# Tilka/hvqm4

Hardware: AMD Instinct MI355X
Metric: decoded Mpixels/s (bit-exact YUV) (higher is better)
Workload: dtype u8

## Files before the change

### hvqm4_amd/csrc/hvq_kernels.hip

```cpp
#include <hip/hip_runtime.h>
#include <stdint.h>
#include <algorithm>

#include "hvq_desc.h"
#include "../../include/hvqm4_amd.h"

typedef uint32_t u32;
typedef int32_t i32;
typedef uint64_t __attribute__((aligned(1))) u64u;
#define GLB __attribute__((address_space(1)))
typedef short s16x2 __attribute__((ext_vector_type(2)));
typedef unsigned short u16x2 __attribute__((ext_vector_type(2)));

#define HVQ_WG HVQ_TILE_BLOCKS
#ifndef HVQ_MIN_WAVES
#define HVQ_MIN_WAVES 8
#endif

struct Blk { u32 r[4]; };

__device__ __forceinline__ u32 sat_pack(s16x2 a, s16x2 b)
{
    const u16x2 k255 = { 255, 255 };
    u16x2 ua = __builtin_elementwise_min(__builtin_bit_cast(u16x2, (s16x2)(a >> 3)), k255);
// ... 27 lines not shown
#pragma unroll
    for (int y = 0; y < 4; ++y) r.q[y] = *(const GLB u64u *)(ref + a + y * stride);
    r.q[4] = 0;
    if (hy) r.q[4] = *(const GLB u64u *)(ref + a + 4 * stride);
    return r;
}

__device__ __forceinline__ Blk mc_filter(const McRows &rows, int hx, int hy)
{
    const uint64_t *q = rows.q;
    Blk o;
    u32 hp, xp;
    {
        const u32 p = (u32)q[0], n = hx ? (u32)(q[0] >> 8) : p;
        hp = __builtin_amdgcn_lerp(p, n, 0u); xp = p ^ n;
    }
#pragma unroll
    for (int y = 0; y < 4; ++y) {
        const u32 p = (u32)q[y + 1], n = hx ? (u32)(q[y + 1] >> 8) : p;
        const u32 hn = __builtin_amdgcn_lerp(p, n, 0u), xn = p ^ n;
        const u32 h1 = hy ? hn : hp, x1 = hy ? xn : xp;
        const u32 t = __builtin_amdgcn_lerp(hp, h1, 0x01010101u);
        o.r[y] = t + (xp & x1 & ~(hp ^ h1) & 0x01010101u);
        hp = hn; xp = xn;
    }
    return o;
}


template <int N>
__device__ __forceinline__ u32 udiv_table(u32 den)
{
    const u32 q = (u32)__builtin_fmaf(__builtin_amdgcn_rcpf((float)den), (float)N, 0.0009765625f);
    return den ? q : 0u;
}

__device__ __forceinline__ i32 sar(u32 v, i32 s)
{
    i32 r = (i32)v >> s;
    __asm__ volatile("" : "+v"(r));
    return r;
}

__device__ __forceinline__ u32 basis_gain(u32 d, u32 lo, u32 hi)
{
    const u32 q = udiv_table<256>((hi - lo) & 15u);
    const u32 s = d >> 14;
    const u32 g = s * (q << 4);
    return (d & 0x2000u) ? 0u - g : g;
}

template <int STRIDE>
__device__ __forceinline__ void basis_scatter(u32 g, const u32 e[16], u32 *acc_lds)
{
#if defined(HVQ_ABL) && HVQ_ABL == 5
    u32 t = 0;
#pragma unroll
    for (int i = 0; i < 16; ++i) t ^= g * e[i];
    __hip_atomic_fetch_add(acc_lds, t, __ATOMIC_RELAXED, __HIP_MEMORY_SCOPE_WORKGROUP);
#else
#pragma unroll
    for (int i = 0; i < 16; ++i)
        __hip_atomic_fetch_add(acc_lds + i * STRIDE, g * e[i], __ATOMIC_RELAXED, __HIP_MEMORY_SCOPE_WORKGROUP);
#endif
}

__device__ __forceinline__ u32 shr_sat_pack4(u32 a, u32 b, u32 c, u32 d, i32 s)
{
    const u32 lo = (u32)__builtin_amdgcn_ashr_pk_u8_i32((i32)a, (i32)b, (u32)s);
    const u32 hi = (u32)__builtin_amdgcn_ashr_pk_u8_i32((i32)c, (i32)d, (u32)s);
    return __builtin_amdgcn_perm(hi, lo, 0x05040100u);
}

__device__ __forceinline__ Blk intra_finish(const u32 r[16], i32 V, i32 unk)
{
    u32 total = 0;
#pragma unroll
    for (int i = 0; i < 16; ++i) total += r[i];
    const u32 delta = ((u32)V << unk) - (u32)((i32)total >> 4);
    Blk o4;
#pragma unroll
    for (int y = 0; y < 4; ++y)
        o4.r[y] = shr_sat_pack4(r[4 * y] + delta, r[4 * y + 1] + delta, r[4 * y + 2] + delta, r[4 * y + 3] + delta, unk);
    return o4;
}

__device__ __forceinline__ Blk predi_finish(const u32 r[16], Blk m, u32 p0, u32 p1, i32 unk)
{
    u32 total = 0;
#pragma unroll
    for (int i = 0; i < 16; ++i) total += r[i];
    const u32 mean_aot = (u32)((i32)total >> 4);
    u32 sum = 8;
#pragma unroll
    for (int y = 0; y < 4; ++y) sum = __builtin_amdgcn_sad_u8(m.r[y], 0u, sum);
    const u32 mean = sum >> 4;
    u32 lo = 255, hi = 0;
#pragma unroll
    for (int y = 0; y < 4; ++y)
#pragma unroll
        for (int x = 0; x < 4; ++x) {
            const u32 v = (m.r[y] >> (8 * x)) & 0xFFu;
            lo = min(lo, v);
            hi = max(hi, v);
        }
    const u32 mcd = udiv_table<4096>(hi - lo);
    const u32 factor = p1 * mcd;
    const u32 c = p0 - mean_aot - mean * factor;
    Blk o4;
#pragma unroll
    for (int y = 0; y < 4; ++y) {
        u32 v[4];
#pragma unroll
        for (int x = 0; x < 4; ++x) {
            const u32 px = (m.r[y] >> (8 * x)) & 0xFFu;
            v[x] = (u32)(((i32)(r[4 * y + x] + c + px * factor) >> unk) + (i32)px);
        }
        o4.r[y] = shr_sat_pack4(v[0], v[1], v[2], v[3], 0);
    }
    return o4;
}

__device__ __forceinline__ u32 wave_incl_scan(u32 v)
{
    v += (u32)__builtin_amdgcn_update_dpp(0, (int)v, 0x111, 0xF, 0xF, false);
    v += (u32)__builtin_amdgcn_update_dpp(0, (int)v, 0x112, 0xF, 0xF, false);
    v += (u32)__builtin_amdgcn_update_dpp(0, (int)v, 0x114, 0xF, 0xF, false);
    v += (u32)__builtin_amdgcn_update_dpp(0, (int)v, 0x118, 0xF, 0xF, false);
    v += (u32)__builtin_amdgcn_update_dpp(0, (int)v, 0x142, 0xA, 0xF, false);
    v += (u32)__builtin_amdgcn_update_dpp(0, (int)v, 0x143, 0xC, 0xF, false);
    return v;
}

__device__ __forceinline__ u32 lanes_below(unsigned long long mask)
{
    return __builtin_amdgcn_mbcnt_hi((u32)(mask >> 32), __builtin_amdgcn_mbcnt_lo((u32)mask, 0u));
}

#define HVQ_NW (HVQ_WG / 64)
#ifndef HVQ_ABL
#define HVQ_ABL 0
#endif
#ifndef HVQ_NT_LOADS
#define HVQ_NT_LOADS 0
#endif
#ifndef HVQ_PRIO
#define HVQ_PRIO 0
#endif
#ifndef HVQ_PLANE_LOAD
#define HVQ_PLANE_LOAD 1
#endif
#ifndef HVQ_NT_STORES
#define HVQ_NT_STORES 1
#endif

#ifdef HVQ_STAMPS
static unsigned long long *g_stamps = nullptr;
extern "C" __attribute__((visibility("default"))) void hvq_set_stamps(unsigned long long *p) { g_stamps = p; }
#define HVQ_STAMP_ARG , unsigned long long *stamps
#define STAMP(i, VM) do { unsigned long long t_; __builtin_amdgcn_sched_barrier(0); \
        if (VM) asm volatile("s_waitcnt vmcnt(0)" ::: "memory"); \
        asm volatile("s_memtime %0\n\ts_waitcnt lgkmcnt(0)" : "=s"(t_) :: "memory"); __builtin_amdgcn_sched_barrier(0); \
        if (stamps && (threadIdx.x & 63) == 0) stamps[(((size_t)blockIdx.z * gridDim.y + blockIdx.y) * gridDim.x + blockIdx.x) * 64 + (threadIdx.x >> 6) * 16 + (i)] = t_; } while (0)
#else
#define HVQ_STAMP_ARG
#define STAMP(i, VM) do { } while (0)
#endif

typedef u32 u32x2 __attribute__((ext_vector_type(2)));
#define HVQ_PIN(x) do { x = (u32)__builtin_amdgcn_readfirstlane((int)(x)); asm("" : "+s"(x)); } while (0)

struct SrGeo {
    GLB uint8_t *pic;
    i32 lim;
};
__device__ __forceinline__ u32 sr_ld(const SrGeo &g, i32 o)
{
    o = clampi(o, 0, g.lim);
    return __hip_atomic_load(g.pic + o, __ATOMIC_RELAXED, __HIP_MEMORY_SCOPE_AGENT);
}
__device__ __forceinline__ void sr_st(const SrGeo &g, i32 o, u32 v)
{
    o = clampi(o, 0, g.lim);
    __hip_atomic_store(g.pic + o, (uint8_t)v, __ATOMIC_RELAXED, __HIP_MEMORY_SCOPE_AGENT);
}
__device__ __forceinline__ u32 sr_mc_sample(const SrGeo &g, i32 so, i32 stride, int hx, int hy, int i, int j)
{
    const i32 a = so + i * stride + j;
    if (!hx && !hy) return sr_ld(g, a);
    if (hx && !hy) return (sr_ld(g, a) + sr_ld(g, a + 1) + 1u) / 2u;
    if (!hx) return (sr_ld(g, a) + sr_ld(g, a + stride) + 1u) / 2u;
    return (sr_ld(g, a) + sr_ld(g, a + 1) + sr_ld(g, a + stride) + sr_ld(g, a + stride + 1) + 2u) >> 2;
}

__global__ __launch_bounds__(HVQ_WG)
void hvq_selfref_kernel(const HvqJob *__restrict__ J, const uint8_t *__restrict__ side, uint8_t *pic)
{
    const int tid = threadIdx.x;
    const u32 flags = J->flags;
    const bool is15 = flags & HVQ_F_IS15, landscape = flags & HVQ_F_LANDSCAPE;
    const i32 unk = (i32)((flags >> HVQ_JOB_UNK_SHIFT) & 31u);
    const i32 lw = (i32)J->width, mcb_w = (i32)J->mcb_w;
    const i32 nmb = mcb_w * (i32)((J->plane[0].hbvb >> 16) / 2u);
    const GLB u32 *__restrict__ pool = (const GLB u32 *)J->pool;
    const GLB u32 *__restrict__ mvs = (const GLB u32 *)J->mv;
    const GLB u32 *__restrict__ offs = (const GLB u32 *)((const GLB uint8_t *)J->tq + J->q_offs_off);
    SrGeo g;
    g.pic = (GLB uint8_t *)pic;
    g.lim = (i32)J->slot_bytes - 1;
    struct { const GLB uint8_t *map; i32 hb, pw, ws, hs, poff; u32 tile_first; } P[3];
#pragma unroll
    for (int k = 0; k < 3; ++k) {
        P[k].map = (const GLB uint8_t *)J->plane[k].map;
        P[k].hb = (i32)(J->plane[k].hbvb & 0xFFFFu);
        P[k].pw = (i32)(J->plane[k].pw_sub & 0xFFFFu);
        P[k].ws = (i32)((J->plane[k].pw_sub >> 16) & 0xFFu); P[k].hs = (i32)(J->plane[k].pw_sub >> 24);
        P[k].poff = (i32)J->plane[k].plane_off;
        P[k].tile_first = J->plane[k].tile_first;
    }
    bool moved = false;
    for (i32 m = 0; m < nmb; ++m) {
        const i32 my = m / mcb_w, mx = m - my * mcb_w;
        const u32 T = (u32)__builtin_amdgcn_readfirstlane((int)P[0].map[2 * ((2 * my + 1) * (P[0].hb + 2) + 2 * mx + 1) + 1]);
        if (((T >> 5) & 3u) != 2u) {
            int k = -1, r = 0, col = 0;
            const int cw = 8 >> P[1].ws, ch = 8 >> P[1].hs, cn = cw * ch;
            if (tid < 64) { k = 0; r = tid >> 3; col = tid & 7; }
            else if (tid - 64 < cn) { k = 1; r = (tid - 64) / cw; col = (tid - 64) - r * cw; }
            else if (tid - 64 - cn < cn) { k = 2; r = (tid - 64 - cn) / cw; col = (tid - 64 - cn) - r * cw; }
            if (k >= 0) {
                const i32 o = P[k].poff + (my * (8 >> P[k].hs) + r) * P[k].pw + mx * (8 >> P[k].ws) + col;
                pic[o] = side[o];
            }
            moved = true;
            continue;
        }
        if (moved) { __syncthreads(); moved = false; }
        if (tid == 0) {
            const u32 mvw = mvs[m];
            const i32 rx = (i32)(int16_t)(mvw & 0xFFFF), ry = (i32)(int16_t)(mvw >> 16);
            const bool proc = T & 0x10u;
            const i32 origin = landscape ? rx / 2 + (ry / 2 - 16) * lw - 32 : rx / 2 + (ry / 2 - 32) * lw - 16;
            for (int k = 0; k < 3; ++k) {
                const i32 pw = P[k].pw, ws = P[k].ws, hs = P[k].hs;
                const i32 pdx = rx >> ws, pdy = ry >> hs;
                const int hx = is15 ? (pdx & 1) : (rx & 1), hy = is15 ? (pdy & 1) : (ry & 1);
                const int bxp = 2 >> ws, byp = 2 >> hs, nblk = bxp * byp;
                for (int j = 0; j < nblk; ++j) {
                    const int dx = nblk == 1 ? 0 : (j >> 1), dy = nblk == 1 ? 0 : ((j == 1 || j == 2) ? 1 : 0);
                    const i32 bx = mx * bxp + dx, by = my * byp + dy;
                    const i32 dsto = P[k].poff + by * 4 * pw + bx * 4;
                    const i32 srco = P[k].poff + (pdy >> 1) * pw + (pdx >> 1) + dy * 4 * pw + dx * 4;
                    const u32 kind = (u32)P[k].map[2 * ((by + 1) * (P[k].hb + 2) + bx + 1) + 1] & 0xFu;
                    const u32 b = (u32)(by * P[k].hb + bx);
                    const u32 off = offs[(size_t)(P[k].tile_first + b / HVQ_TILE_BLOCKS) * HVQ_TILE_BLOCKS + b % HVQ_TILE_BLOCKS];
                    if (!proc && kind == 6u) {
                        for (int i = 0; i < 4; ++i) {
                            const u32 w4 = pool[off + (u32)i];
                            for (int x = 0; x < 4; ++x) sr_st(g, dsto + i * pw + x, (w4 >> (8 * x)) & 0xFFu);
                        }
                    } else if (proc || kind == 0u) {
                        for (int i = 0; i < 4; ++i)
                            for (int x = 0; x < 4; ++x) sr_st(g, dsto + i * pw + x, sr_mc_sample(g, srco, pw, hx, hy, i, x));
                    } else {
                        u32 acc[16];
                        for (int i = 0; i < 16; ++i) acc[i] = 0;
                        const u32 nb = kind - 1u;
                        for (u32 q = 0; q < nb; ++q) {
                            const u32 d = pool[off + 2u + q];
                            const i32 ol = d & 0x3F, os = (d >> 6) & 0x1F;
                            const u32 sl = (d >> 11) & 1, ss = (d >> 12) & 1;
                            i32 o, ys, xs;
                            if (landscape) { o = lw * os + ol; xs = 1 << sl; ys = lw << ss; }
                            else           { o = lw * ol + os; xs = 1 << ss; ys = lw << sl; }
                            u32 e[16], lo = 255, hi = 0;
                            for (int i = 0; i < 4; ++i)
                                for (int x = 0; x < 4; ++x) {
                                    const u32 v = (sr_ld(g, origin + o + i * ys + x * xs) >> 4) & 15u;
                                    e[4 * i + x] = v; lo = min(lo, v); hi = max(hi, v);
                                }
                            const u32 gn = basis_gain(d, lo, hi);
                            for (int i = 0; i < 16; ++i) acc[i] += gn * e[i];
                        }
                        u32 total = 0;
                        for (int i = 0; i < 16; ++i) total += acc[i];
                        const u32 mean_aot = (u32)((i32)total >> 4);
                        u32 md[16], sum = 8, lo = 255, hi = 0;
                        for (int i = 0; i < 4; ++i)
                            for (int x = 0; x < 4; ++x) { const u32 v = sr_mc_sample(g, srco, pw, hx, hy, i, x); md[4 * i + x] = v; sum += v; lo = min(lo, v); hi = max(hi, v); }
                        const i32 mean = (i32)(sum >> 4);
                        const u32 addend = pool[off] - mean_aot;
                        const u32 factor = pool[off + 1u] * udiv_table<4096>(hi - lo);
                        for (int i = 0; i < 16; ++i) {
                            const u32 t = (u32)((i32)md[i] - mean) * factor;
                            const i32 v = sar(acc[i] + addend + t, unk) + (i32)md[i];
                            sr_st(g, dsto + (i >> 2) * pw + (i & 3), (u32)clampi(v, 0, 255));
                        }
                    }
                }
            }
        }
        __syncthreads();
    }
}

extern "C" hipError_t hvq_launch_selfref(const HvqJob *job_dev, const uint8_t *side, uint8_t *dst, hipStream_t stream)
{
    hipLaunchKernelGGL(hvq_selfref_kernel, dim3(1), dim3(HVQ_WG), 0, stream, job_dev, side, dst);
    return hipGetLastError();
}

__device__ __forceinline__ u32 gain_q(u32 w0, u32 lo, u32 hi)
{
    const u32 q = udiv_table<256>((hi - lo) & 15u);
    const u32 g = (w0 & 0x3FFFFu) * (q << 4);
    return (w0 & HVQ_PQ_NEG) ? 0u - g : g;
}

__device__ __forceinline__ void gather_nest_q(i32 o, bool x2, i32 ys, const uint8_t *s_nest, u32 e[16], u32 &lo, u32 &hi)
{
    const u32 sh = x2 ? 8u : 4u;
    lo = 255; hi = 0;
#pragma unroll
    for (int y = 0; y < 4; ++y) {
        const i32 n = o + y * ys;
        uint64_t q = *(const u64u *)(s_nest + (n >> 1));
        q >>= 4 * (n & 1);
        const u32 w0 = (u32)q;
#pragma unroll
        for (int x = 0; x < 4; ++x) {
            u32 v = (w0 >> (sh * x)) & 15u;
            e[4 * y + x] = v;
            lo = min(lo, v);
            hi = max(hi, v);
        }
    }
}

__device__ __forceinline__ void window_load(const GLB uint8_t *ring, u32 voff, u32 ys, uint64_t q[4])
{
    if (HVQ_ABL == 19) { q[0] = *(const GLB u64u *)(ring + (size_t)voff); q[1] = *(const GLB u64u *)(ring + (size_t)(u32)(voff + ys)); q[2] = q[0] ^ 1; q[3] = q[1] ^ 1; return; }
    if (HVQ_ABL == 20) { q[0] = *(const GLB u64u *)(ring + (size_t)voff); q[1] = q[0] ^ 1; q[2] = q[0] ^ 2; q[3] = q[1] ^ 3; return; }
    if (HVQ_ABL == 21) voff &= 0xFFFFu;
#pragma unroll
    for (int y = 0; y < 4; ++y) q[y] = *(const GLB u64u *)(ring + (size_t)(u32)(voff + (u32)y * ys));
}

__device__ __forceinline__ void window_finish(const uint64_t q[4], bool x2, u32 e[16], u32 &lo, u32 &hi)
{
    const u32 sel = x2 ? 0x06040200u : 0x03020100u;
    lo = 255; hi = 0;
#pragma unroll
    for (int y = 0; y < 4; ++y) {
        u32 w = __builtin_amdgcn_perm((u32)(q[y] >> 32), (u32)q[y], sel);
        w = (w >> 4) & 0x0F0F0F0Fu;
#pragma unroll
        for (int x = 0; x < 4; ++x) {
            u32 v = (w >> (8 * x)) & 0xFFu;
            e[4 * y + x] = v;
            lo = min(lo, v);
            hi = max(hi, v);
        }
    }
}


template <int CTX>
__device__ __forceinline__ void inl_classify(u32 T, bool valid, u32 &cls, u32 &nb, u32 &npay, bool &lit, bool &mc, bool &wdc, bool &flat)
{
    const u32 kind = CTX == 0 ? T : (T & 0xFu);
    const bool k0 = kind == 0u, k6 = kind == 6u, k8 = kind == 8u;
    if (CTX == 2) {
        const bool inter = T & 0x60u, proc = T & 0x10u;
        const bool c1 = valid && !inter && !(k0 | k6 | k8), c2 = valid && inter && !proc && !(k0 | k6);
        lit = valid && k6 && !(inter && proc);
        mc = valid && inter && (proc || !k6); wdc = valid && !inter && k0; flat = valid && !inter && k8;
        cls = c1 ? 1u : c2 ? 2u : 0u;
        nb = c1 ? kind : c2 ? kind - 1u : 0u;
        npay = lit ? 4u : nb + (c2 ? 2u : 0u);
    } else {
        const bool c1 = valid && !(k0 | k6 | k8);
        lit = valid && k6; mc = false; wdc = valid && k0; flat = valid && k8;
        cls = c1 ? 1u : 0u; nb = c1 ? kind : 0u; npay = lit ? 4u : nb;
    }
}

template <int N> struct InlCtx { static constexpr int value = N; };
#define HVQ_W64(i) ((uint64_t)cw[i] | ((uint64_t)cw[(i) + 1] << 32))

constexpr u32 HVQ_INL_NEST_LDS = (HVQ_NESTP_BYTES + 8 + 15) / 16 * 16;
constexpr u32 HVQ_INL_ACC_DW = 16, HVQ_INL_RES_DW = 4, HVQ_INL_REC_DW = 3;
constexpr u32 HVQ_INL_CTR_LDS = 16;
constexpr u32 hvq_inl_static_lds(u32 items_cap)
{
    return HVQ_INL_NEST_LDS + 4u * (HVQ_INL_ACC_DW + HVQ_INL_RES_DW + HVQ_INL_REC_DW) * items_cap + HVQ_INL_CTR_LDS;
}
#ifndef HVQ_SEVEN_WG_CAP
#define HVQ_SEVEN_WG_CAP 128
#endif
constexpr int hvq_inl_waves(int tpw, int items_cap) { return (tpw >= 2 && items_cap >= HVQ_SEVEN_WG_CAP) ? 7 : HVQ_MIN_WAVES; }
template <int ITEMS_CAP, int TPW> struct InlWaves { static constexpr int value = hvq_inl_waves(TPW, ITEMS_CAP); };

template <int ITEMS_CAP, int TPW>
__global__ __launch_bounds__(HVQ_WG, (InlWaves<ITEMS_CAP, TPW>::value))
void hvq_recon_inline_kernel(const HvqJob *__restrict__ jobs, u32 pair_cap, u32 pool_cap HVQ_STAMP_ARG)
{
    extern __shared__ __attribute__((aligned(16))) u32 s_dyn[];
    __shared__ __attribute__((aligned(16))) uint8_t s_nest[HVQ_INL_NEST_LDS];
    __shared__ __attribute__((aligned(16))) u32 s_acc[HVQ_INL_ACC_DW * ITEMS_CAP];
    __shared__ __attribute__((aligned(16))) u32 s_res[HVQ_INL_RES_DW * ITEMS_CAP];
    __shared__ u32 s_item0[ITEMS_CAP];
    __shared__ u32 s_item1[ITEMS_CAP];
    __shared__ u32 s_item2[ITEMS_CAP];
    __shared__ __attribute__((aligned(16))) unsigned long long s_ctr64;
    static_assert(sizeof(s_nest) + sizeof(s_acc) + sizeof(s_res) + sizeof(s_item0) + sizeof(s_item1) + sizeof(s_item2) + HVQ_INL_CTR_LDS == hvq_inl_static_lds(ITEMS_CAP)
                  && ITEMS_CAP % 4 == 0 && sizeof(s_ctr64) <= HVQ_INL_CTR_LDS, "the host sizes launches by hvq_inl_static_lds");
    u32 *const s_pair = s_dyn;
    u32 *const s_pool = s_dyn + pair_cap;

    const int tid = threadIdx.x;
    const u32 lane = (u32)tid & 63u;
    STAMP(0, 0);
#if HVQ_PRIO == 1 || HVQ_PRIO == 2
    __builtin_amdgcn_s_setprio(3);
#endif
    const u32 slot_id = blockIdx.z * gridDim.x + blockIdx.x;
    const u32 wg = blockIdx.y;
    const HvqJob *__restrict__ J = jobs + slot_id;
#if HVQ_PLANE_LOAD
    const u32 *__restrict__ CW = (const u32 *)J;
    u32 cw[20];
#pragma unroll
    for (int i = 0; i < 20; ++i) cw[i] = CW[i];
    u32 wb_lo = CW[46], wb_hi = CW[47], q_offs_off = CW[49];
#pragma unroll
    for (int i = 0; i < 20; ++i) HVQ_PIN(cw[i]);
    HVQ_PIN(wb_lo); HVQ_PIN(wb_hi); HVQ_PIN(q_offs_off);
    const u32 total_tiles = cw[17];
    const u32 n0 = cw[18], n1 = cw[19] - cw[18], n2 = total_tiles - cw[19];
    const u32 pf1 = (n0 + TPW - 1) / TPW, pf2 = pf1 + (n1 + TPW - 1) / TPW, pend = pf2 + (n2 + TPW - 1) / TPW;
    if (total_tiles == 0 || wg >= pend) return;
    const int p = (wg >= pf1) + (wg >= pf2);
    const u32 *__restrict__ PW = CW + 20 + 8 * p;
    u32 w[8];
#pragma unroll
    for (int i = 0; i < 8; ++i) w[i] = PW[i];
    u32 magic = CW[52 + p], magic16 = CW[55 + p];
#pragma unroll
    for (int i = 0; i < 8; ++i) HVQ_PIN(w[i]);
    HVQ_PIN(magic); HVQ_PIN(magic16);
#else
    const u32 *__restrict__ PW = (const u32 *)&J->plane[0];
    u32 w0[8], w1[8], w2[8];
#pragma unroll
    for (int i = 0; i < 8; ++i) { w0[i] = PW[i]; w1[i] = PW[8 + i]; w2[i] = PW[16 + i]; }
    const u32 *__restrict__ CW = (const u32 *)J;
    u32 cw[18];
#pragma unroll
    for (int i = 0; i < 18; ++i) cw[i] = CW[i];
    u32 wb_lo = CW[46], wb_hi = CW[47], q_offs_off = CW[49];
    u32 mg0 = CW[52], mg1 = CW[53], mg2 = CW[54], ms0 = CW[55], ms1 = CW[56], ms2 = CW[57];
#pragma unroll
    for (int i = 0; i < 8; ++i) { HVQ_PIN(w0[i]); HVQ_PIN(w1[i]); HVQ_PIN(w2[i]); }
#pragma unroll
    for (int i = 0; i < 18; ++i) HVQ_PIN(cw[i]);
    HVQ_PIN(wb_lo); HVQ_PIN(wb_hi); HVQ_PIN(q_offs_off);
    HVQ_PIN(mg0); HVQ_PIN(mg1); HVQ_PIN(mg2); HVQ_PIN(ms0); HVQ_PIN(ms1); HVQ_PIN(ms2);
    const u32 total_tiles = cw[17];
    const u32 n0 = w1[5] - w0[5], n1 = w2[5] - w1[5], n2 = total_tiles - w2[5];
    const u32 pf1 = (n0 + TPW - 1) / TPW, pf2 = pf1 + (n1 + TPW - 1) / TPW, pend = pf2 + (n2 + TPW - 1) / TPW;
    if (total_tiles == 0 || wg >= pend) return;
    const int p = (wg >= pf1) + (wg >= pf2);
    u32 w[8];
#pragma unroll
    for (int i = 0; i < 8; ++i) w[i] = p == 0 ? w0[i] : p == 1 ? w1[i] : w2[i];
    const u32 magic = p == 0 ? mg0 : p == 1 ? mg1 : mg2, magic16 = p == 0 ? ms0 : p == 1 ? ms1 : ms2;
#endif
    const u32 hbvb = w[6], pw_sub = w[7], tile_first = w[5];
    const u32 nplane_tiles = p == 0 ? n0 : p == 1 ? n1 : n2;
    const u32 pairw = wg - (p == 0 ? 0u : p == 1 ? pf1 : pf2);
    const u32 tile0 = tile_first + (u32)TPW * pairw;
    const int ntl = TPW == 1 ? 1 : (int)min((u32)TPW, nplane_tiles - (u32)TPW * pairw);
    const uint64_t map_a = (uint64_t)w[0] | ((uint64_t)w[1] << 32);
    const uint64_t dst_a = (uint64_t)w[2] | ((uint64_t)w[3] << 32);
    const u32 plane_off = w[4];
    const u32 hb = hbvb & 0xFFFFu;
    const u32 flags = cw[13];
    const u32 pic_kind = (flags >> HVQ_JOB_KIND_SHIFT) & 3u;
    const i32 unk = (i32)((flags >> HVQ_JOB_UNK_SHIFT) & 31u);
    const bool is_pb = pic_kind != HVQ_PIC_I;
    const bool landscape = flags & HVQ_F_LANDSCAPE;
    const bool is15 = flags & HVQ_F_IS15;
    const u32 nblocks = hb * (hbvb >> 16);
    const u32 b0 = (u32)TPW * pairw * HVQ_TILE_BLOCKS;
    const u32 ws = (pw_sub >> 16) & 0xFFu, hs = pw_sub >> 24;
    const u32 pw = pw_sub & 0xFFFFu;
    const u32 mstride = hb + 2u;
    const GLB uint8_t *map = (const GLB uint8_t *)map_a;
    const GLB uint8_t *ring = (const GLB uint8_t *)HVQ_W64(0);
    const u32 ref0_off = cw[2], ref1_off = cw[3];
    const GLB u32 *__restrict__ pool = (const GLB u32 *)HVQ_W64(4);
    const GLB u32 *__restrict__ mvs = (const GLB u32 *)HVQ_W64(6);
    const GLB uint8_t *__restrict__ qb = (const GLB uint8_t *)HVQ_W64(8);
    const GLB u32 *__restrict__ nestp = (const GLB u32 *)HVQ_W64(10);
    const GLB u32 *__restrict__ wave_base = (const GLB u32 *)((uint64_t)wb_lo | ((uint64_t)wb_hi << 32));
    GLB uint8_t *plane = (GLB uint8_t *)dst_a;
    const i32 slot = (i32)cw[12];
    const u32 lw = cw[14];
    const u32 mcb_w = cw[15];
    const u32 pool_dwords = cw[16];
    const u32 wave = (u32)__builtin_amdgcn_readfirstlane(tid >> 6);
    STAMP(1, 0);
    if (tid == 0) s_ctr64 = 0;
    __syncthreads();

    u32 plo = wave_base[tile0 * HVQ_NW];
    u32 phi = tile0 + (u32)ntl < total_tiles ? wave_base[(tile0 + (u32)ntl) * HVQ_NW] : pool_dwords;
    u32 wbase[TPW];
#pragma unroll
    for (int h = 0; h < TPW; ++h) wbase[h] = h < ntl ? wave_base[(tile0 + (u32)h) * HVQ_NW + wave] : 0u;
    bool valid[TPW];
    u32 bx[TPW], by[TPW];
    uint64_t row8[TPW];
    u32 nt[TPW], nbt[TPW], mvw[TPW];
    Blk blk[TPW];
    u32 doff[TPW], rslot[TPW];
#pragma unroll
    for (int h = 0; h < TPW; ++h) {
        const u32 bw = b0 + (u32)(h * HVQ_TILE_BLOCKS) + wave * 64u;
        const bool livew = h < ntl && bw < nblocks;
        valid[h] = h < ntl && bw + lane < nblocks;
        const u32 bws = livew ? bw : 0u;
        u32 by0 = __umulhi(bws, magic);
        if ((i32)(bws - by0 * hb) < 0) by0 -= 1u;
        const u32 bx0 = bws - by0 * hb;
        const u32 l = valid[h] ? lane : 0u;
        const u32 t = bx0 + l;
        u32 q;
        if (hb >= 64u) q = t >= hb ? 1u : 0u;
        else q = __umul24(t, magic16) >> 16;
        bx[h] = t - __umul24(q, hb); by[h] = by0 + q;
        doff[h] = valid[h] ? __umul24(by[h] << 2, pw) + (bx[h] << 2) : 0xFFFFFFFFu;
        const GLB uint8_t *mw = map + 2u * (size_t)(bws + 2u * by0 + hb + 3u);
        const u32 vo2 = 2u * (l + 2u * q);
#if HVQ_NT_LOADS
        row8[h] = __builtin_nontemporal_load((const GLB u64u *)((mw - 2) + vo2));
#else
        row8[h] = *(const GLB u64u *)((mw - 2) + vo2);
#endif
        if (HVQ_ABL >= 41 && HVQ_ABL <= 43) { nt[h] = (u32)row8[h] & 0xFFFFu; nbt[h] = (u32)(row8[h] >> 32) & 0xFFFFu; }
        else { nt[h] = *(const GLB uint16_t *)((mw - 2u * (size_t)mstride) + vo2); nbt[h] = *(const GLB uint16_t *)((mw + 2u * (size_t)mstride) + vo2); }
        mvw[h] = 0;
        if (HVQ_ABL == 42 || HVQ_ABL == 43) { if (is_pb) { const u32 hh = ((bx[h] >> (1u - ws)) * 73u + (by[h] >> (1u - hs)) * 151u) * 2654435761u; mvw[h] = (((hh >> 8) & 1023u) + 16u) | ((((hh >> 18) & 511u) + 64u) << 16); } }
        else if (is_pb) mvw[h] = *(const GLB u32 *)((const GLB uint8_t *)mvs + 4u * (__umul24(by[h] >> (1u - hs), mcb_w) + (bx[h] >> (1u - ws))));
    }
    typedef __attribute__((address_space(3))) u32 lds_u32;
    const bool has_nest = (HVQ_W64(10) != 0) && HVQ_ABL != 43;
    if (has_nest) {
        constexpr u32 NCH = HVQ_NESTP_BYTES / 16u;
        static_assert(HVQ_NESTP_BYTES % 16 == 0, "nest in 16-byte pieces");
#pragma unroll
        for (u32 r0 = 0; r0 < NCH; r0 += HVQ_WG)
            if (r0 + (u32)tid < NCH)
                __builtin_amdgcn_global_load_lds((const GLB u32 *)((const GLB uint8_t *)nestp + 16u * (r0 + (u32)tid)), (lds_u32 *)((u32 *)s_nest + 4u * (r0 + wave * 64u)), 16, 0, 0);
    }
    phi = max(phi, plo);
    const u32 plo4 = plo & ~3u;
    const u32 nst = HVQ_ABL == 43 ? 0u : min(phi - plo4, pool_cap);
    {
        const GLB uint8_t *pool_lo = (const GLB uint8_t *)(pool + plo4);
        const u32 nch = (nst + 3u) >> 2;
        for (u32 r0 = 0; r0 < nch; r0 += HVQ_WG)
            if (r0 + (u32)tid < nch) __builtin_amdgcn_global_load_lds((const GLB u32 *)(pool_lo + 16u * (r0 + (u32)tid)), (lds_u32 *)(s_pool + 4u * (r0 + wave * 64u)), 16, 0, 0);
    }
    const u32 nst_lim = phi - plo4 <= pool_cap ? 0xFFFFFFFFu : nst;
    auto pool_at = [&](u32 idx) -> u32 {
        const u32 j = idx - plo4;
        return j < nst_lim ? s_pool[j] : pool[min(idx, pool_dwords ? pool_dwords - 1u : 0u)];
    };

#if HVQ_PRIO == 1
    __builtin_amdgcn_s_setprio(0);
#endif
    STAMP(2, 0);
    STAMP(3, 1);
    auto front = [&](auto ctxc) {
        constexpr int CTX = decltype(ctxc)::value;
        u32 off[TPW], cls[TPW], nb[TPW], e16v[TPW], w0v[TPW], pinI[TPW], pinM[TPW], npayv[TPW];
        bool lit[TPW], mcb[TPW], wdcb[TPW], flatb[TPW], hxb[TPW], hyb[TPW];
        unsigned long long m1[TPW], m2[TPW];
        McRows rows[TPW];
#pragma unroll
        for (int h = 0; h < TPW; ++h) {
            const u32 e16 = (u32)(row8[h] >> 16) & 0xFFFFu;
            const u32 T = e16 >> 8, V = e16 & 0xFFu;
            e16v[h] = e16;
            u32 npay;
            inl_classify<CTX>(T, valid[h], cls[h], nb[h], npay, lit[h], mcb[h], wdcb[h], flatb[h]);
            npayv[h] = npay;
            if (HVQ_ABL == 36 || HVQ_ABL == 37) { cls[h] = 0; nb[h] = 0; }
            w0v[h] = 0; hxb[h] = false; hyb[h] = false;
            if (CTX == 2) {
                const i32 rx = (i32)(int16_t)(mvw[h] & 0xFFFFu), ry = (i32)mvw[h] >> 16;
                const u32 roff = (T & 0x60u) == 0x20u ? ref0_off : ref1_off;
                const u32 hsx = is15 ? ws : 0u, hsy = is15 ? hs : 0u;
                hxb[h] = (rx >> hsx) & 1; hyb[h] = (ry >> hsy) & 1;
                const i32 rowi = HVQ_ABL == 38 ? (i32)(by[h] << 2) : (ry >> (hs + 1u)) + (i32)((by[h] & (1u - hs)) << 2);
                const i32 coli = (HVQ_ABL == 38 ? (i32)(bx[h] << 2) : (rx >> (ws + 1u)) + (i32)((bx[h] & (1u - ws)) << 2)) + (i32)plane_off;
                i32 a = __mul24(rowi, (i32)pw) + coli;
                const i32 hi3 = slot - 8 - 3 * (i32)pw, hi4 = hi3 - (i32)pw;
                a = clampi(a, 0, hyb[h] ? hi4 : hi3);
                if (mcb[h]) w0v[h] = roff + (u32)a;
            }
        }
        if (CTX == 2) {
#pragma unroll
            for (int h = 0; h < TPW; ++h) {
                if (mcb[h]) {
                    const u32 vo = w0v[h];
                    if (HVQ_ABL == 34 || HVQ_ABL == 37) {
#pragma unroll
                        for (int y = 0; y < 5; ++y) rows[h].q[y] = (uint64_t)vo * 0x0101010101ull + (uint64_t)y;
                        continue;
                    }
#pragma unroll
                    for (int y = 0; y < 4; ++y) rows[h].q[y] = *(const GLB u64u *)(ring + (size_t)(u32)(vo + (u32)y * pw));
                    rows[h].q[4] = 0;
                    if (hyb[h]) rows[h].q[4] = *(const GLB u64u *)(ring + (size_t)(u32)(vo + 4u * pw));
                }
            }
        }
#if HVQ_PRIO == 2
        __builtin_amdgcn_s_setprio(0);
#endif
#pragma unroll
        for (int h = 0; h < TPW; ++h) {
            const u32 V = e16v[h] & 0xFFu;
            const u32 npay = npayv[h];
            if (wdcb[h]) {
                const u32 nlf = (u32)row8[h] & 0xFFFFu, nr = (u32)(row8[h] >> 32) & 0xFFFFu;
                const u32 Tt = (nt[h] & 0x7700u) ? V : (nt[h] & 0xFFu);
                const u32 Bb = (nbt[h] & 0x7700u) ? V : (nbt[h] & 0xFFu);
                const u32 Rr = (nr & 0x7700u) ? V : (nr & 0xFFu);
                const bool lexp = CTX == 2 ? !(nlf & 0x7700u) : ((nlf >> 8) & ~8u) == 0u;
                const u32 Ll = lexp ? (nlf & 0xFFu) : V;
                w0v[h] = Tt | (Bb << 8) | (Ll << 16) | (Rr << 24);
            }
            m1[h] = __ballot(cls[h] == 1); m2[h] = CTX == 2 ? __ballot(cls[h] == 2) : 0ull;
            if (CTX == 2) {
                const u32 inc = wave_incl_scan(npay + (nb[h] << (cls[h] == 1 ? 11 : 21)));
                off[h] = wbase[h] + (inc & 0x7FFu) - npay;
                pinI[h] = (inc >> 11) & 0x3FFu; pinM[h] = inc >> 21;
            } else {
                const u32 inc = wave_incl_scan(npay + (nb[h] << 16));
                off[h] = wbase[h] + (inc & 0xFFFFu) - npay;
                pinI[h] = inc >> 16; pinM[h] = 0;
            }
        }
        STAMP(4, 0);
        if (q_offs_off) {
#pragma unroll
            for (int h = 0; h < TPW; ++h)
                if (h < ntl) ((GLB u32 *)(qb + q_offs_off))[(size_t)(tile0 + (u32)h) * HVQ_TILE_BLOCKS + (u32)tid] = off[h];
        }

        u32 slotq[TPW], pstart[TPW];
#pragma unroll
        for (int h = 0; h < TPW; ++h) {
            const u32 c1 = (u32)__popcll(m1[h]), c2 = (u32)__popcll(m2[h]);
            const u32 np1 = (u32)__builtin_amdgcn_readlane((int)pinI[h], 63), np2 = CTX == 2 ? (u32)__builtin_amdgcn_readlane((int)pinM[h], 63) : 0u;
            u32 b1 = 0, b2 = 0, bp1 = 0, bp2 = 0;
            if (c1 | c2) {
                unsigned long long got = 0;
                if (lane == 0)
                    got = __hip_atomic_fetch_add(&s_ctr64, (unsigned long long)c1 | ((unsigned long long)c2 << 10) | ((unsigned long long)np1 << 20) | ((unsigned long long)np2 << 42),
                                                 __ATOMIC_RELAXED, __HIP_MEMORY_SCOPE_WORKGROUP);
                const u32 glo = (u32)__builtin_amdgcn_readfirstlane((int)(u32)got), ghi = (u32)__builtin_amdgcn_readfirstlane((int)(u32)(got >> 32));
                b1 = glo & 1023u; b2 = (glo >> 10) & 1023u;
                bp1 = (glo >> 20) | ((ghi & 1023u) << 12); bp2 = ghi >> 10;
            }
            if (CTX == 2) {
                slotq[h] = cls[h] == 1 ? b1 + lanes_below(m1[h]) : (u32)ITEMS_CAP - 1u - (b2 + lanes_below(m2[h]));
                pstart[h] = cls[h] == 1 ? bp1 + pinI[h] - nb[h] : bp2 + pinM[h] - nb[h];
            } else {
                slotq[h] = b1 + lanes_below(m1[h]);
                pstart[h] = bp1 + pinI[h] - nb[h];
            }
            rslot[h] = cls[h] && slotq[h] < (u32)ITEMS_CAP ? slotq[h] : 0xFFFFFFFFu;
        }
        {
            typedef u32 u32x4z __attribute__((ext_vector_type(4)));
#pragma unroll
            for (u32 i = (u32)tid; i < 4u * ITEMS_CAP; i += HVQ_WG) ((u32x4z *)s_acc)[i] = (u32x4z)(0u);
        }
#pragma unroll
        for (int h = 0; h < TPW; ++h) {
            if (cls[h] && slotq[h] < (u32)ITEMS_CAP) {
                s_item0[slotq[h]] = (u32)(h * HVQ_WG + tid) | (e16v[h] << 10);
                s_item1[slotq[h]] = off[h];
                const bool up = CTX != 2 || cls[h] == 1;
                if (!up) s_item2[slotq[h]] = mvw[h];
                const u32 ent0 = slotq[h] | ((off[h] + (up ? 0u : 2u)) << 9);
                const u32 room = max(pair_cap, pstart[h]) - pstart[h];
                const u32 kmax = min(nb[h], room);
                const u32 pos = up ? pstart[h] : room - kmax;
                const u32 val = up ? ent0 : ent0 + (kmax << 9) - 512u;
                const u32 dv = up ? 512u : 0u - 512u;
                u32 *const sp = s_pair + pos;
#pragma unroll
                for (u32 j = 0; j < 5; ++j)
                    if (j < kmax) sp[j] = val + j * dv;
                if (kmax > 5u) {
#pragma clang loop unroll(disable) vectorize(disable)
                    for (u32 j = 5; j < kmax; ++j) sp[j] = val + j * dv;
                }
            }
        }

#if HVQ_PRIO == 4
        __builtin_amdgcn_s_setprio(3);
#endif
        STAMP(5, 0);
        STAMP(6, 1);
#pragma unroll
        for (int h = 0; h < TPW; ++h) {
            const i32 V = (i32)(e16v[h] & 0xFFu);
            Blk o;
            if (HVQ_ABL == 31 && (mcb[h] || wdcb[h])) {
                o.r[0] = (u32)rows[h].q[0] ^ w0v[h]; o.r[1] = (u32)rows[h].q[1]; o.r[2] = (u32)rows[h].q[2]; o.r[3] = (u32)(rows[h].q[3] ^ rows[h].q[4]);
            } else if (CTX == 2 && mcb[h]) {
                o = mc_filter(rows[h], hxb[h], hyb[h]);
            } else if (wdcb[h]) {
                const u32 nb4 = w0v[h];
                o = weight_block(V, (i32)(nb4 & 0xFF), (i32)((nb4 >> 8) & 0xFF), (i32)((nb4 >> 16) & 0xFF), (i32)(nb4 >> 24));
            } else if (flatb[h]) {
                const u32 v = (u32)V * 0x01010101u;
                o.r[0] = o.r[1] = o.r[2] = o.r[3] = v;
            } else {
                o.r[0] = o.r[1] = o.r[2] = o.r[3] = 0;
            }
            blk[h] = o;
            if (CTX == 2 && cls[h] == 2 && rslot[h] != 0xFFFFFFFFu) {
#pragma unroll
                for (int y = 0; y < 4; ++y) s_res[y * ITEMS_CAP + (int)rslot[h]] = o.r[y];
            }
        }
        STAMP(7, 0);
        __builtin_amdgcn_s_waitcnt(0x0F70);
        __syncthreads();
        STAMP(8, 0);
#pragma unroll
        for (int h = 0; h < TPW; ++h)
            if (lit[h]) {
#pragma unroll
                for (int y = 0; y < 4; ++y) blk[h].r[y] = pool_at(off[h] + (u32)y);
            }
    };
    if (is_pb) front(InlCtx<2>{});
    else if (p == 0) front(InlCtx<0>{});
    else front(InlCtx<1>{});

    const unsigned long long ctr = s_ctr64;
    const u32 nI = min((u32)ctr & 1023u, (u32)ITEMS_CAP), nP = min((u32)(ctr >> 10) & 1023u, (u32)ITEMS_CAP - nI);
    const u32 npI = (u32)(ctr >> 20) & 0x3FFFFFu, npM = (u32)(ctr >> 42);
    const u32 nitems = nI + nP;
    const bool serial = npI + npM > pair_cap;
    const u32 npairs = (serial || HVQ_ABL == 33) ? 0u : npI + npM;

    if (nitems) {
        const i32 nstride = landscape ? 70 : 38;
        auto do_basis = [&](u32 it, u32 d) {
            const i32 ol = d & 0x3F, os = (d >> 6) & 0x1F;
            const u32 sl = (d >> 11) & 1, ss = (d >> 12) & 1;
            const bool x2 = landscape ? sl : ss;
            const u32 y2 = landscape ? ss : sl;
            const u32 wq0 = (d >> 14) | ((d & 0x2000u) ? HVQ_PQ_NEG : 0u);
            u32 e[16], lo, hi;
            if (it >= nI) {
                const u32 t16 = s_item0[it] >> 10;
                const u32 roff = ((t16 >> 13) & 3u) == 1u ? ref0_off : ref1_off;
                const i32 o = landscape ? (i32)lw * os + ol : (i32)lw * ol + os;
                const i32 ys = (i32)lw << y2;
                const u32 mv = s_item2[it];
                const i32 rx = (i32)(int16_t)(mv & 0xFFFFu), ry = (i32)mv >> 16;
                const i32 rx2 = (rx - (rx >> 31)) >> 1, ry2 = (ry - (ry >> 31)) >> 1;
                const i32 origin = __mul24(ry2, (i32)lw) + rx2 - (landscape ? 16 * (i32)lw + 32 : 32 * (i32)lw + 16);
                const u32 voff = roff + (u32)clampi(origin + o, 0, slot - 8 - 3 * ys);
                uint64_t wq[4];
                window_load(ring, voff, (u32)ys, wq);
                window_finish(wq, x2, e, lo, hi);
            } else {
                const i32 o = landscape ? nstride * os + ol : nstride * ol + os;
                gather_nest_q(o, x2, nstride << y2, s_nest, e, lo, hi);
            }
            basis_scatter<ITEMS_CAP>(gain_q(wq0, lo, hi), e, s_acc + it);
        };
        if (!serial) {
            const bool psplit = npairs <= (u32)HVQ_WG;
            for (u32 v = (u32)tid; v < (psplit ? (u32)HVQ_WG : npairs); v += HVQ_WG) {
                u32 pi;
                if (psplit) {
                    const u32 back = (u32)(HVQ_WG - 1) - v;
                    if (v < npI) pi = v;
                    else if (back < npM) pi = pair_cap - 1u - back;
                    else continue;
                } else pi = v < npI ? v : pair_cap - 1u - (v - npI);
                const u32 pr = s_pair[pi];
                do_basis(pr & 511u, pool_at(pr >> 9));
            }
        } else {
            for (u32 v = (u32)tid; v < nitems; v += HVQ_WG) {
                const u32 it = v < nI ? v : (u32)ITEMS_CAP - 1u - (v - nI);
                const u32 q16 = s_item0[it] >> 10;
                const u32 kind = (q16 >> 8) & ((is_pb || p != 0) ? 0xFu : 0xFFu);
                const bool item_mc = v >= nI;
                const u32 n = item_mc ? (kind & 0xFu) - 1u : kind;
                const u32 bases = s_item1[it] + (item_mc ? 2u : 0u);
                for (u32 k = 0; k < n; ++k) do_basis(it, pool_at(bases + k));
            }
        }
        STAMP(9, 1);
        __syncthreads();
        STAMP(10, 0);
        const bool split = nitems <= (u32)HVQ_WG;
        for (u32 v = (u32)tid; v < (split ? (u32)HVQ_WG : nitems); v += HVQ_WG) {
            bool item_mc;
            u32 it;
            if (split) {
                const u32 back = (u32)(HVQ_WG - 1) - v;
                item_mc = v < nP;
                if (!item_mc && back >= nI) continue;
                it = item_mc ? (u32)ITEMS_CAP - 1u - v : back;
            } else {
                item_mc = v >= nI;
                it = v < nI ? v : (u32)ITEMS_CAP - 1u - (v - nI);
            }
            const u32 item = s_item0[it];
            const u32 q16 = item >> 10;
            const u32 poff = s_item1[it];
            u32 r[16];
#pragma unroll
            for (int i = 0; i < 16; ++i) r[i] = s_acc[i * ITEMS_CAP + it];
            u32 *const so = s_res + it;
            Blk o;
            if (HVQ_ABL == 32) {
                o.r[0] = r[0] ^ poff; o.r[1] = r[5]; o.r[2] = r[10]; o.r[3] = r[15] ^ q16;
            } else if (item_mc) {
                Blk m;
#pragma unroll
                for (int y = 0; y < 4; ++y) m.r[y] = so[y * ITEMS_CAP];
                o = predi_finish(r, m, pool_at(poff), pool_at(poff + 1u), unk);
            } else {
                o = intra_finish(r, (i32)(q16 & 0xFF), unk);
            }
#pragma unroll
            for (int y = 0; y < 4; ++y) so[y * ITEMS_CAP] = o.r[y];
        }
    }
    STAMP(11, 0);
#if HVQ_PRIO == 3
    __builtin_amdgcn_s_setprio(3);
#endif
    __syncthreads();
    STAMP(12, 0);

#pragma unroll
    for (int h = 0; h < TPW; ++h)
        if (rslot[h] != 0xFFFFFFFFu) {
#pragma unroll
            for (int y = 0; y < 4; ++y) blk[h].r[y] = s_res[y * ITEMS_CAP + (int)rslot[h]];
        }
    if ((HVQ_ABL == 35 || HVQ_ABL == 37) && blk[0].r[0] != 0x12345678u) return;
    constexpr bool WIDE = ITEMS_CAP < HVQ_SEVEN_WG_CAP;
    static_assert(!WIDE || HVQ_INL_ACC_DW * ITEMS_CAP >= 4 * HVQ_WG, "a wave's 64 blocks of 16 bytes pass through the accumulators");
    if (WIDE && (hb & 3u) == 0) {
        auto wave_sync = [] {
            __builtin_amdgcn_fence(__ATOMIC_RELEASE, "wavefront");
            __builtin_amdgcn_wave_barrier();
            __builtin_amdgcn_fence(__ATOMIC_ACQUIRE, "wavefront");
        };
        u32 *const tw = s_acc + wave * 256u;
        const u32 g4 = 4u * (lane & 15u), rr = lane >> 4;
#pragma unroll
        for (int h = 0; h < TPW; ++h) {
#pragma unroll
            for (int y = 0; y < 4; ++y) tw[y * 64 + (int)lane] = blk[h].r[y];
            wave_sync();
            const u32 d0 = (u32)__builtin_amdgcn_ds_bpermute((int)(g4 << 2), (int)doff[h]);
            typedef u32 u32x4 __attribute__((ext_vector_type(4)));
            const u32x4 v = *(const u32x4 *)&tw[rr * 64u + g4];
            wave_sync();
            if (d0 == 0xFFFFFFFFu) continue;
            const u32 a = d0 + __umul24(rr, pw);
#if HVQ_NT_STORES
            if (HVQ_NT_STORES == 2 || pic_kind == HVQ_PIC_B) asm volatile("global_store_dwordx4 %0, %1, %2 nt" :: "v"(a), "v"(v), "s"(plane) : "memory");
            else
#endif
                *(GLB u32x4 *)(plane + (size_t)a) = v;
        }
    } else
#pragma unroll
    for (int h = 0; h < TPW; ++h) {
        if (doff[h] == 0xFFFFFFFFu) continue;
#if HVQ_NT_STORES
        if (HVQ_NT_STORES == 2 || pic_kind == HVQ_PIC_B) {
#pragma unroll
            for (int y = 0; y < 4; ++y) asm volatile("global_store_dword %0, %1, %2 nt" :: "v"(doff[h] + (u32)y * pw), "v"(blk[h].r[y]), "s"(plane) : "memory");
        } else
#endif
        {
#pragma unroll
            for (int y = 0; y < 4; ++y) *(GLB u32 *)(plane + (size_t)(doff[h] + (u32)y * pw)) = blk[h].r[y];
        }
    }
    STAMP(13, 0);
    STAMP(14, 1);
}

template <int ITEMS_CAP, int TPW>
static void launch_recon_inline(const HvqJob *jobs_dev, uint32_t nslots, uint32_t max_wgs, uint32_t pair_cap, uint32_t pool_cap, hipStream_t stream)
{
    const dim3 grid = nslots >= 8 ? dim3(8, max_wgs, nslots / 8) : dim3(nslots, max_wgs, 1);
    static const size_t lds_pad = getenv("HVQM4_AMD_LDS_PAD") ? (size_t)atoi(getenv("HVQM4_AMD_LDS_PAD")) : 0;
#ifdef HVQ_STAMPS
    hipLaunchKernelGGL((hvq_recon_inline_kernel<ITEMS_CAP, TPW>), grid, dim3(HVQ_WG), (size_t)(pair_cap + pool_cap) * 4u + lds_pad, stream, jobs_dev, pair_cap, pool_cap, g_stamps);
#else
    hipLaunchKernelGGL((hvq_recon_inline_kernel<ITEMS_CAP, TPW>), grid, dim3(HVQ_WG), (size_t)(pair_cap + pool_cap) * 4u + lds_pad, stream, jobs_dev, pair_cap, pool_cap);
#endif
}

extern "C" __attribute__((visibility("default"))) uint32_t hvq_recon_inline_dyn_lds(uint32_t pair_cap, uint32_t pool_cap)
{
    return 4u * (((std::max(pair_cap, 1u) + 3u) & ~3u) + ((pool_cap + 3u) & ~3u));
}

extern "C" __attribute__((visibility("default"))) uint32_t hvq_recon_inline_max_wgs(uint32_t tiles_per_wg, uint32_t items_cap)
{
    return (uint32_t)hvq_inl_waves((int)tiles_per_wg, (int)std::min(items_cap, 512u));
}

extern "C" __attribute__((visibility("default"))) uint32_t hvq_recon_inline_static_lds(uint32_t tiles_per_wg, uint32_t items_cap)
{
    (void)tiles_per_wg;
    return hvq_inl_static_lds(items_cap);
}

extern "C" hipError_t hvq_launch_recon_inline(const HvqJob *jobs_dev, uint32_t nslots, uint32_t max_wgs, uint32_t tiles_per_wg,
                                              uint32_t items_cap, uint32_t pair_cap, uint32_t pool_cap, hipStream_t stream)
{
    if (nslots == 0 || max_wgs == 0) return hipSuccess;
    pair_cap = (std::max(pair_cap, 1u) + 3u) & ~3u;
    pool_cap = (pool_cap + 3u) & ~3u;
// ... 641 lines not shown
```

Before: 696,000.

## Hoist first-round motion-comp basis window loads ahead of block reconstruction

For P/B frames, a new path moves the barrier earlier, reads each thread's first basis pair and issues its four reference-window loads before the per-block reconstruction work. The loaded rows are finished and scattered later, and the main pair loop then skips that first round. This is meant to hide global-memory latency of the motion-compensated basis gathers behind the front-end compute. It adds an explicit vmcnt wait and carries extra live registers (four 64-bit values plus the item and descriptor) across the front stage, which may raise register pressure.

```diff
diff --git a/hvqm4_amd/csrc/hvq_kernels.hip b/hvqm4_amd/csrc/hvq_kernels.hip
--- a/hvqm4_amd/csrc/hvq_kernels.hip
+++ b/hvqm4_amd/csrc/hvq_kernels.hip
@@ -203,6 +203,9 @@
 #endif
 #ifndef HVQ_NT_STORES
 #define HVQ_NT_STORES 1
+#endif
+#ifndef HVQ_GATHER_SPLIT
+#define HVQ_GATHER_SPLIT 1
 #endif
 
 #ifdef HVQ_STAMPS
@@ -390,15 +393,18 @@
 
 __device__ __forceinline__ void window_load(const GLB uint8_t *ring, u32 voff, u32 ys, uint64_t q[4])
 {
-    if (HVQ_ABL == 19) { q[0] = *(const GLB u64u *)(ring + (size_t)voff); q[1] = *(const GLB u64u *)(ring + (size_t)(u32)(voff + ys)); q[2] = q[0] ^ 1; q[3] = q[1] ^ 1; return; }
-    if (HVQ_ABL == 20) { q[0] = *(const GLB u64u *)(ring + (size_t)voff); q[1] = q[0] ^ 1; q[2] = q[0] ^ 2; q[3] = q[1] ^ 3; return; }
+    if (HVQ_ABL == 19) { q[0] = *(const GLB u64u *)(ring + (size_t)voff); q[1] = *(const GLB u64u *)(ring + (size_t)(u32)(voff + ys)); q[2] = q[3] = 0; return; }
+    if (HVQ_ABL == 20) { q[0] = *(const GLB u64u *)(ring + (size_t)voff); q[1] = q[2] = q[3] = 0; return; }
     if (HVQ_ABL == 21) voff &= 0xFFFFu;
 #pragma unroll
     for (int y = 0; y < 4; ++y) q[y] = *(const GLB u64u *)(ring + (size_t)(u32)(voff + (u32)y * ys));
 }
 
-__device__ __forceinline__ void window_finish(const uint64_t q[4], bool x2, u32 e[16], u32 &lo, u32 &hi)
-{
+__device__ __forceinline__ void window_finish(const uint64_t qin[4], bool x2, u32 e[16], u32 &lo, u32 &hi)
+{
+    uint64_t q[4] = { qin[0], qin[1], qin[2], qin[3] };
+    if (HVQ_ABL == 19) { q[2] = q[0] ^ 1; q[3] = q[1] ^ 1; }
+    if (HVQ_ABL == 20) { q[1] = q[0] ^ 1; q[2] = q[0] ^ 2; q[3] = q[1] ^ 3; }
     const u32 sel = x2 ? 0x06040200u : 0x03020100u;
     lo = 255; hi = 0;
 #pragma unroll
@@ -630,6 +636,25 @@
         return j < nst_lim ? s_pool[j] : pool[min(idx, pool_dwords ? pool_dwords - 1u : 0u)];
     };
 
+    constexpr bool GSPLIT = HVQ_GATHER_SPLIT && TPW >= 2 && ITEMS_CAP >= HVQ_SEVEN_WG_CAP;
+    auto window_origin = [&](u32 it, u32 d, u32 &voff, u32 &ysu) {
+        const i32 ol = d & 0x3F, os = (d >> 6) & 0x1F;
+        const u32 sl = (d >> 11) & 1, ss = (d >> 12) & 1;
+        const u32 y2 = landscape ? ss : sl;
+        const u32 t16 = s_item0[it] >> 10;
+        const u32 roff = ((t16 >> 13) & 3u) == 1u ? ref0_off : ref1_off;
+        const i32 o = landscape ? (i32)lw * os + ol : (i32)lw * ol + os;
+        const i32 ys = (i32)lw << y2;
+        const u32 mv = s_item2[it];
+        const i32 rx = (i32)(int16_t)(mv & 0xFFFFu), ry = (i32)mv >> 16;
+        const i32 rx2 = (rx - (rx >> 31)) >> 1, ry2 = (ry - (ry >> 31)) >> 1;
+        const i32 origin = __mul24(ry2, (i32)lw) + rx2 - (landscape ? 16 * (i32)lw + 32 : 32 * (i32)lw + 16);
+        voff = roff + (u32)clampi(origin + o, 0, slot - 8 - 3 * ys);
+        ysu = (u32)ys;
+    };
+    u32 rq_it = 0xFFFFFFFFu, rq_d = 0;
+    uint64_t rq_q[4] = { 0, 0, 0, 0 };
+
 #if HVQ_PRIO == 1
     __builtin_amdgcn_s_setprio(0);
 #endif
@@ -664,6 +689,8 @@
                 if (mcb[h]) w0v[h] = roff + (u32)a;
             }
         }
+        constexpr bool GS = GSPLIT && CTX == 2;
+        if (GS) asm volatile("s_waitcnt vmcnt(0)" ::: "memory");
         if (CTX == 2) {
 #pragma unroll
             for (int h = 0; h < TPW; ++h) {
@@ -773,6 +800,35 @@
 #endif
         STAMP(5, 0);
         STAMP(6, 1);
+        if (GS) {
+            asm volatile("s_waitcnt lgkmcnt(0)\n\ts_barrier" ::: "memory");
+            STAMP(8, 0);
+            const unsigned long long ctr = s_ctr64;
+            const u32 nI = min((u32)ctr & 1023u, (u32)ITEMS_CAP);
+            const u32 npI = (u32)(ctr >> 20) & 0x3FFFFFu, npM = (u32)(ctr >> 42);
+            const bool none = npI + npM > pair_cap || HVQ_ABL == 33;
+            const u32 qI = none ? 0u : npI, qM = none ? 0u : npM;
+            const bool psplit = qI + qM <= (u32)HVQ_WG;
+            const u32 back = (u32)(HVQ_WG - 1) - (u32)tid;
+            const bool act = !psplit || (u32)tid < qI || back < qM;
+            const u32 pi = (u32)tid < qI ? (u32)tid : pair_cap - 1u - (psplit ? back : (u32)tid - qI);
+            u32 voff = 0, ys = 0;
+            if (act) {
+                const u32 pr = s_pair[pi];
+                const u32 it = pr & 511u, j = (pr >> 9) - plo4;
+                u32 d;
+                if (j < nst_lim) d = s_pool[j];
+                else {
+                    d = pool[min(pr >> 9, pool_dwords ? pool_dwords - 1u : 0u)];
+                    asm volatile("" : "+v"(d));
+                }
+                rq_it = it; rq_d = d;
+                if (it >= nI) window_origin(it, d, voff, ys);
+            }
+            if (HVQ_ABL != 33) window_load(ring, voff, ys, rq_q);
+            __builtin_amdgcn_sched_barrier(0);
+            STAMP(15, 0);
+        }
 #pragma unroll
         for (int h = 0; h < TPW; ++h) {
             const i32 V = (i32)(e16v[h] & 0xFFu);
@@ -797,9 +853,11 @@
             }
         }
         STAMP(7, 0);
-        __builtin_amdgcn_s_waitcnt(0x0F70);
-        __syncthreads();
-        STAMP(8, 0);
+        if (!GS) {
+            __builtin_amdgcn_s_waitcnt(0x0F70);
+            __syncthreads();
+            STAMP(8, 0);
+        }
 #pragma unroll
         for (int h = 0; h < TPW; ++h)
             if (lit[h]) {
@@ -820,35 +878,44 @@
 
     if (nitems) {
         const i32 nstride = landscape ? 70 : 38;
+        auto basis_fields = [&](u32 d, bool &x2, u32 &wq0) {
+            const u32 sl = (d >> 11) & 1, ss = (d >> 12) & 1;
+            x2 = landscape ? sl : ss;
+            wq0 = (d >> 14) | ((d & 0x2000u) ? HVQ_PQ_NEG : 0u);
+        };
+        auto nest_basis = [&](u32 d, bool x2, u32 e[16], u32 &lo, u32 &hi) {
+            const i32 ol = d & 0x3F, os = (d >> 6) & 0x1F;
+            const u32 y2 = landscape ? (d >> 12) & 1 : (d >> 11) & 1;
+            const i32 o = landscape ? nstride * os + ol : nstride * ol + os;
+            gather_nest_q(o, x2, nstride << y2, s_nest, e, lo, hi);
+        };
         auto do_basis = [&](u32 it, u32 d) {
-            const i32 ol = d & 0x3F, os = (d >> 6) & 0x1F;
-            const u32 sl = (d >> 11) & 1, ss = (d >> 12) & 1;
-            const bool x2 = landscape ? sl : ss;
-            const u32 y2 = landscape ? ss : sl;
-            const u32 wq0 = (d >> 14) | ((d & 0x2000u) ? HVQ_PQ_NEG : 0u);
-            u32 e[16], lo, hi;
+            bool x2;
+            u32 wq0, e[16], lo, hi;
+            basis_fields(d, x2, wq0);
             if (it >= nI) {
-                const u32 t16 = s_item0[it] >> 10;
-                const u32 roff = ((t16 >> 13) & 3u) == 1u ? ref0_off : ref1_off;
-                const i32 o = landscape ? (i32)lw * os + ol : (i32)lw * ol + os;
-                const i32 ys = (i32)lw << y2;
-                const u32 mv = s_item2[it];
-                const i32 rx = (i32)(int16_t)(mv & 0xFFFFu), ry = (i32)mv >> 16;
-                const i32 rx2 = (rx - (rx >> 31)) >> 1, ry2 = (ry - (ry >> 31)) >> 1;
-                const i32 origin = __mul24(ry2, (i32)lw) + rx2 - (landscape ? 16 * (i32)lw + 32 : 32 * (i32)lw + 16);
-                const u32 voff = roff + (u32)clampi(origin + o, 0, slot - 8 - 3 * ys);
+                u32 voff, ys;
                 uint64_t wq[4];
-                window_load(ring, voff, (u32)ys, wq);
+                window_origin(it, d, voff, ys);
+                window_load(ring, voff, ys, wq);
                 window_finish(wq, x2, e, lo, hi);
             } else {
-                const i32 o = landscape ? nstride * os + ol : nstride * ol + os;
-                gather_nest_q(o, x2, nstride << y2, s_nest, e, lo, hi);
+                nest_basis(d, x2, e, lo, hi);
             }
             basis_scatter<ITEMS_CAP>(gain_q(wq0, lo, hi), e, s_acc + it);
         };
+        const bool first_done = GSPLIT && is_pb;
+        if (first_done && rq_it != 0xFFFFFFFFu) {
+            bool x2;
+            u32 wq0, e[16], lo, hi;
+            basis_fields(rq_d, x2, wq0);
+            if (rq_it >= nI) window_finish(rq_q, x2, e, lo, hi);
+            else nest_basis(rq_d, x2, e, lo, hi);
+            basis_scatter<ITEMS_CAP>(gain_q(wq0, lo, hi), e, s_acc + rq_it);
+        }
         if (!serial) {
             const bool psplit = npairs <= (u32)HVQ_WG;
-            for (u32 v = (u32)tid; v < (psplit ? (u32)HVQ_WG : npairs); v += HVQ_WG) {
+            for (u32 v = (u32)tid + (first_done ? (u32)HVQ_WG : 0u); v < (psplit ? (u32)HVQ_WG : npairs); v += HVQ_WG) {
                 u32 pi;
                 if (psplit) {
                     const u32 back = (u32)(HVQ_WG - 1) - v;
```

Result: no change. 700,800, median of 6 (+0.7%).
